# ZongyueQin/SessionSimilaritySearch

Hardware: AMD Instinct MI355X
Metric: session queries/sec (higher is better)
Workload: dtype f32

## Files before the change

### sessionsimilaritysearch_amd/_lib.py

```python
from __future__ import annotations

import ctypes
import os
import subprocess
from ctypes import c_float, c_int, c_int32, c_int64, c_size_t, c_void_p

_HERE = os.path.dirname(os.path.abspath(__file__))
LIB_PATH = os.path.join(_HERE, "libsss.so")
CSRC = os.path.join(_HERE, "csrc")

_lib = None

_SIGNATURES = {
    "sss_version": (c_int, []),
    "sss_last_error": (ctypes.c_char_p, []),
    "sss_normalize_rows": (c_int, [c_void_p, c_int64, c_int, c_int64, c_float, c_int, c_void_p]),
    "sss_row_norm_max": (c_int, [c_void_p, c_int64, c_int, c_int, c_void_p, c_void_p]),
    "sss_f32_to_bf16": (c_int, [c_void_p, c_int64, c_void_p, c_void_p]),
    "sss_ip_topk_workspace_bytes": (c_size_t, [c_int64, c_int64, c_int, c_int, c_int]),
    "sss_ip_topk_state_bytes": (c_size_t, [c_int64]),
    "sss_ip_topk": (c_int, [c_void_p, c_int64, c_void_p, c_int64, c_int, c_int, c_int, c_int64, c_float,
                            c_void_p, c_void_p, c_void_p, c_void_p, c_void_p, c_size_t, c_void_p, c_size_t, c_void_p]),
    "sss_split_bf16": (c_int, [c_void_p, c_int64, c_int, c_void_p, c_void_p]),
    "sss_ip_topk_split": (c_int, [c_void_p, c_int64, c_void_p, c_void_p, c_int64, c_int, c_int, c_int64, c_float,
# ... 80 lines not shown
_SPARSE_SIGNATURES = {
    "sss_session_vectors_count": (c_int, [c_void_p, c_void_p, c_void_p, c_int64, c_int64, c_void_p, c_void_p, c_void_p]),
    "sss_session_vectors_fill": (c_int, [c_void_p, c_void_p, c_void_p, c_int64, c_int64, c_int, ctypes.c_double, c_void_p, c_void_p,
                                         c_void_p, c_void_p, c_void_p]),
    "sss_sparse_topk_workspace_bytes": (c_size_t, [c_int64, c_int64]),
    "sss_sparse_topk": (c_int, [c_void_p, c_void_p, c_void_p, c_int64, c_void_p, c_void_p, c_void_p, c_int64, c_int, c_int64,
                                c_void_p, c_void_p, c_void_p, c_size_t, c_void_p]),
}

_L2_SIGNATURES = {
    "sss_l2_row_bias": (c_int, [c_void_p, c_int64, c_int, c_void_p, c_void_p]),
    "sss_l2_topk_workspace_bytes": (c_size_t, [c_int64, c_int64, c_int, c_int, c_int]),
    "sss_l2_topk": (c_int, [c_void_p, c_int64, c_void_p, c_void_p, c_int, c_int, c_float, c_void_p, c_int64, c_int, c_int, c_int64,
                            c_float, c_void_p, c_void_p, c_void_p, c_void_p, c_void_p, c_size_t, c_void_p, c_size_t, c_void_p]),
    "sss_l2_topk_threshold_workspace_bytes": (c_size_t, [c_int64, c_int64, c_int, c_int]),
    "sss_l2_topk_threshold": (c_int, [c_void_p, c_void_p, c_int64, c_void_p, c_void_p, c_int, c_int, c_float, c_void_p, c_int64, c_int,
                                      c_int, c_int64, c_float, c_void_p, c_void_p, c_void_p, c_void_p, c_size_t, c_void_p]),
}

_L2_LONG_SIGNATURES = {
    "sss_l2_topk_long_workspace_bytes": (c_size_t, [c_int64, c_int64, c_int]),
    "sss_l2_topk_long": (c_int, [c_void_p, c_int64, c_void_p, c_void_p, c_int, c_float, c_void_p, c_int64, c_int, c_int, c_int64,
                                 c_float, c_void_p, c_void_p, c_void_p, c_void_p, c_size_t, c_void_p]),
}

_PAD_SIGNATURES = {
    "sss_pad_rows_f32": (c_int, [c_void_p, c_int64, c_int, c_int, c_void_p, c_void_p]),
    "sss_pad_scale_f16": (c_int, [c_void_p, c_int64, c_int, c_int, c_int, c_void_p, c_void_p]),
    "sss_pad_split_bf16": (c_int, [c_void_p, c_int64, c_int, c_int, c_void_p, c_void_p]),
    "sss_pad_f16_resid_max": (c_int, [c_void_p, c_void_p, c_int64, c_int, c_int, c_int, c_void_p, c_void_p]),
    "sss_pad_topk_workspace_bytes": (c_size_t, [c_int64, c_int64, c_int, c_int, c_int, c_int]),
    "sss_pad_topk": (c_int, [c_void_p, c_int64, c_void_p, c_void_p, c_int, c_int, c_float, c_void_p, c_int64, c_int, c_int, c_int,
                             c_int64, c_float, c_void_p, c_void_p, c_void_p, c_void_p, c_void_p, c_size_t, c_void_p, c_size_t,
                             c_void_p]),
    "sss_pad_topk_threshold_workspace_bytes": (c_size_t, [c_int64, c_int64, c_int, c_int, c_int]),
    "sss_pad_topk_threshold": (c_int, [c_void_p, c_void_p, c_int64, c_void_p, c_void_p, c_int, c_int, c_float, c_void_p, c_int64,
                                       c_int, c_int, c_int, c_int64, c_float, c_void_p, c_void_p, c_void_p, c_void_p, c_size_t,
                                       c_void_p]),
}

GRAPH_IGNORE_QUERY = 1
_GRAPH_SIGNATURES = {
    "sss_graph_counts_ex": (c_int, [c_void_p, c_void_p, c_void_p, c_int64, c_int, c_void_p, c_void_p, c_void_p, c_void_p]),
    "sss_graph_fill_ex": (c_int, [c_void_p, c_void_p, c_void_p, c_void_p, c_int64, c_int, c_void_p, c_void_p, c_void_p, c_void_p,
                                  c_void_p]),
}

_EVAL_SIGNATURES = {
    "sss_item_overlap": (c_int, [c_void_p, c_void_p, c_int64, c_void_p, c_void_p, c_int64, c_void_p, c_int, c_int64, c_void_p, c_void_p,
                                 c_void_p, c_void_p]),
    "sss_overlap_metrics": (c_int, [c_void_p, c_void_p, c_void_p, c_int64, c_int, c_float, c_void_p, c_void_p, c_void_p]),
}


HEADERS = {
    "sss.h": _SIGNATURES,
    "sss_sparse.h": _SPARSE_SIGNATURES,
    "sss_l2.h": _L2_SIGNATURES,
    "sss_l2_long.h": _L2_LONG_SIGNATURES,
    "sss_pad.h": _PAD_SIGNATURES,
    "sss_graph.h": _GRAPH_SIGNATURES,
    "sss_eval.h": _EVAL_SIGNATURES,
}


class LinearProblem(ctypes.Structure):
    _fields_ = [("x", c_void_p), ("ldx", c_int64), ("ids", c_void_p), ("table", c_void_p), ("xcopy", c_void_p),
                ("ld_xcopy", c_int64), ("w", c_void_p), ("ldw", c_int64), ("bias", c_void_p), ("y", c_void_p),
                ("ldy", c_int64), ("n", c_int64), ("m", c_int32), ("act", c_int32), ("post_scale", c_void_p), ("post_shift", c_void_p)]


class GraphOut(ctypes.Structure):
    _fields_ = [(n, c_void_p) for n in ("q_x", "q_batch", "q_pos", "p_x", "p_batch", "p_cnt", "rowptr_qp", "col_qp",
                                        "rowptr_pq", "col_pq", "rowptr_pp", "col_pp", "w_pp", "src_row", "pos_id")]


class LayerArgs(ctypes.Structure):
    _fields_ = [("yp", c_void_p), ("ld_yp", c_int64), ("yq", c_void_p), ("ld_yq", c_int64), ("h", c_int32), ("d_x", c_int32),
                ("rowptr_qp", c_void_p), ("col_qp", c_void_p), ("rowptr_pp", c_void_p), ("col_pp", c_void_p),
                ("w_pp", c_void_p), ("bias_qp", c_void_p), ("b_ih", c_void_p),
                ("xin_p", c_void_p), ("ld_xin", c_int64), ("out_p", c_void_p), ("ld_out_p", c_int64), ("np", c_int64),
                ("rowptr_pq", c_void_p), ("col_pq", c_void_p), ("bias_pq", c_void_p),
                ("out_q", c_void_p), ("ld_out_q", c_int64), ("nq", c_int64), ("n_self_loop", c_int64),
                ("row_p", c_void_p), ("row_q", c_void_p), ("x0_p", c_void_p), ("ld_x0_p", c_int64),
                ("xq_table", c_void_p), ("ld_xq", c_int64), ("x0_q", c_void_p), ("ld_x0_q", c_int64)]


def exported_symbols():
    return sorted(HEADERS["sss.h"])


def sparse_symbols():
    return sorted(HEADERS["sss_sparse.h"])


def l2_symbols():
    return sorted(HEADERS["sss_l2.h"])


def l2_long_symbols():
    return sorted(HEADERS["sss_l2_long.h"])


def pad_symbols():
    return sorted(HEADERS["sss_pad.h"])


def graph_symbols():
    return sorted(HEADERS["sss_graph.h"])


def eval_symbols():
    return sorted(HEADERS["sss_eval.h"])


def build(verbose: bool = False) -> str:
    cmd = ["make", "-C", CSRC, "-j4"]
    res = subprocess.run(cmd, capture_output=True, text=True)
    if res.returncode != 0:
        raise RuntimeError("building libsss.so failed:\n" + res.stdout[-4000:] + res.stderr[-4000:])
    if verbose:
        print(res.stdout)
    return LIB_PATH


def lib():
    global _lib
    if _lib is None:
        if not os.path.exists(LIB_PATH):
            raise RuntimeError(
                f"{LIB_PATH} is missing: the HIP extension is not built. Run "
                "`python -c 'import __graft_entry__ as g; g.build()'` (or `make -C "
                "sessionsimilaritysearch_amd/csrc`). There is no CPU fallback.")
        h = ctypes.CDLL(LIB_PATH)
        for table in HEADERS.values():
            for name, (res, args) in table.items():
                fn = getattr(h, name)
                fn.restype, fn.argtypes = res, args
        _lib = h
    return _lib


class SssError(RuntimeError):
    pass


def check(rc: int, what: str):
    if rc != 0:
        msg = lib().sss_last_error()
        raise SssError(f"{what} failed (rc={rc}): {msg.decode() if msg else ''}")


def stream_ptr(device=None):
    import torch
    return torch.cuda.current_stream(device).cuda_stream


def require_cuda(t, name, dtype=None):
    import torch
    if not isinstance(t, torch.Tensor) or not t.is_cuda:
        raise SssError(f"{name} must be a CUDA (HIP) tensor")
    if dtype is not None and t.dtype != dtype:
        raise SssError(f"{name} must have dtype {dtype}, got {t.dtype}")
    if not t.is_contiguous():
        raise SssError(f"{name} must be contiguous")
    return t
# ... 1 lines not shown
```

### sessionsimilaritysearch_amd/csrc/ip_topk.hip

```cpp
#include "scan.h"

namespace sss {

namespace {
constexpr int PROF_RING = 512;
struct Prof {
    bool on = false;
    int n = 0;
    hipEvent_t ev[2 * PROF_RING];
    bool made = false;
};
Prof g_prof[MAX_DEVICES];
}

extern "C" int sss_profile_enable(int on) {
    Prof& p = g_prof[current_device()];
    if (on && !p.made) {
        for (int i = 0; i < 2 * PROF_RING; ++i)
            if (hipEventCreate(&p.ev[i]) != hipSuccess) { set_error("profile_enable: hipEventCreate failed"); return SSS_EHIP; }
        p.made = true;
    }
    p.on = on != 0;
    p.n = 0;
    return SSS_OK;
// ... 48 lines not shown
    t.scan_dtype = scan_dtype; t.corpus_shift = corpus_shift; t.corpus_resid = corpus_resid; t.corpus_max_norm = corpus_max_norm;
    t.id_offset = id_offset;
    return t;
}

extern "C" size_t sss_ip_topk_state_bytes(int64_t nq) { return nq > 0 ? state_words(nq) * 4 : 0; }

extern "C" size_t sss_ip_topk_workspace_bytes(int64_t nq, int64_t n, int d, int k, int dtype) {
    if (nq <= 0 || n <= 0 || k <= 0 || !corpus_dtype_ok(dtype) || !fused_shape_ok(d, dtype)) return 0;
    return make_plan(nq, n, d, k, dtype).total_bytes;
}

static size_t ip_topk_scan_workspace_bytes(long nq, long n, int d, int k, int scan_dtype) {
    if (nq <= 0 || n <= 0 || k <= 0 || !fused_shape_ok(d, scan_dtype)) return 0;
    return make_plan(nq, n, d, k, scan_dtype).total_bytes;
}

extern "C" size_t sss_ip_topk_f16_workspace_bytes(int64_t nq, int64_t n, int d, int k) {
    return ip_topk_scan_workspace_bytes(nq, n, d, k, DT_F16);
}

extern "C" int sss_f16_shift(float amax) { return f16_shift(amax); }

static int ip_topk_impl(const char* what, const void* q, long nq, const void* c_scan, int scan_dtype, int corpus_shift,
                        float corpus_resid, const void* c_exact,
                        int exact_dtype, long n, int d, int k, long id_offset, float corpus_max_norm, float* D_out, long* I_out,
                        int* status, int* unproven_count, void* state, size_t state_bytes, void* ws, size_t ws_bytes,
                        hipStream_t st, const float* bias = nullptr, int d_row = 0) {
    const bool l2 = bias != nullptr;
    if (nq <= 0 || n <= 0 || k <= 0) { set_error("%s: nq, n, k must be positive", what); return SSS_EINVAL; }
    int rc = check_scan_source(what, exact_dtype, scan_dtype, d, false, c_scan, corpus_shift, corpus_resid, n, nq);
    if (rc) return rc;
    if (k > 500) { set_error("%s: k too large (max 500)", what); return SSS_EINVAL; }
    if ((reinterpret_cast<uintptr_t>(ws) & 255) || (reinterpret_cast<uintptr_t>(state) & 15)) {
        set_error("%s: workspace must be 256-byte aligned, state 16-byte aligned", what);
        return SSS_EINVAL;
    }
    if (!state || state_bytes < sss_ip_topk_state_bytes(nq)) { set_error("%s: state %zu < %zu bytes", what, state_bytes, sss_ip_topk_state_bytes(nq)); return SSS_EWORKSPACE; }
    const ScanPlan p = make_plan(nq, n, d, k, scan_dtype);
    if (ws_bytes < p.total_bytes) { set_error("%s: workspace %zu < %zu", what, ws_bytes, p.total_bytes); return SSS_EWORKSPACE; }
    char* w = reinterpret_cast<char*>(ws);

    ScanArgs a;
    a.Q = q; a.C = c_scan; a.nq = (int)nq; a.n = (int)n;
    a.tiles_per_split = p.tiles_per_split; a.total_tiles = p.total_tiles;
    a.S = p.S; a.G = p.G; a.J = p.J; a.Ju = p.Ju; a.cert = p.cert; a.boot = p.boot; a.append = p.append; a.cap = p.cap;
    a.tau_skip = p.tau_skip;
    unsigned* sw = reinterpret_cast<unsigned*>(state);
    a.slots = sw;
    a.cnt = sw + state_off_cnt(nq);
    a.maxlast = reinterpret_cast<unsigned long long*>(sw + state_off_maxlast(nq));
    a.cand = reinterpret_cast<unsigned long long*>(w);
    a.bias = bias; a.corpus_shift = corpus_shift;
    Prof& pr = g_prof[current_device()];
    const bool prof = pr.on && pr.n < PROF_RING;
    if (prof) (void)hipEventRecord(pr.ev[2 * pr.n], st);
    rc = launch_scan(scan_dtype, d, p.tile_rows, a, st);
    if (prof) { (void)hipEventRecord(pr.ev[2 * pr.n + 1], st); ++pr.n; }
    if (rc) return rc;

    SelectArgs s;
    s.Q = q; s.C = c_exact; s.nq = (int)nq; s.d = d; s.dtype = exact_dtype; s.scan_dtype = scan_dtype; s.corpus_shift = corpus_shift; s.corpus_resid = corpus_resid;
    s.k = k; s.K2 = p.K2; s.J = p.J; s.cap = p.cap; s.tau_skip = p.tau_skip;
    s.cand = a.cand; s.slots = a.slots; s.cnt = a.cnt; s.maxlast = a.maxlast;
    s.id_offset = id_offset; s.corpus_max_norm = corpus_max_norm;
    s.D_out = D_out; s.I_out = I_out; s.status = status; s.unproven_count = unproven_count;
    s.metric = l2 ? 1 : 0;
    s.d_row = d_row;
    rc = launch_select(s, st);
    if (rc) (void)hipMemsetAsync(state, 0, sss_ip_topk_state_bytes(nq), st);
    return rc;
}

template <class Prepare, class Select>
static int run_threshold_form(const ThrArgs& t, const void* c_scan, const ScanPlan& p, Prepare prepare, Select select, hipStream_t st,
                              const float* bias = nullptr) {
    int rc = prepare();
    if (rc) return rc;
    ScanArgs a = {};
    a.Q = t.Q; a.C = c_scan; a.nq = t.nsel; a.n = (int)t.n;
    a.tiles_per_split = p.tiles_per_split; a.total_tiles = p.total_tiles;
    a.S = p.S; a.G = p.G; a.J = 0; a.Ju = 0; a.cert = 1; a.boot = 0; a.append = 0; a.cap = p.cap;
    a.slots = nullptr; a.cnt = t.cnt; a.maxlast = nullptr;
    a.cand = const_cast<unsigned long long*>(t.cand);
    a.qsel = t.qsel; a.thr = t.thr;
    a.bias = bias; a.corpus_shift = t.corpus_shift;
    rc = launch_scan(t.scan_dtype, t.d, p.tile_rows, a, st);
    if (rc) return rc;
    return select();
}

constexpr int THR_CAP = 8192;
static size_t thr_head_bytes(long nsel) { return ((size_t)nsel * 8 + 255) & ~(size_t)255; }

extern "C" size_t sss_ip_topk_threshold_workspace_bytes(int64_t nsel, int64_t n, int d, int scan) {
    if (nsel <= 0 || n <= 0 || !fused_shape_ok(d, scan)) return 0;
    return thr_head_bytes(nsel) + make_thr_plan(nsel, n, d, scan, THR_CAP).total_bytes;
}

static int topk_threshold_impl(const char* what, const void* q, const int* qsel, long nsel, const void* c_exact, int exact_dtype,
                               const void* c_scan, int scan_dtype, int corpus_shift, float corpus_resid, long n, int d, int k,
                               long id_offset, float corpus_max_norm, float* D_out, long* I_out, int* status, void* ws, size_t ws_bytes,
                               hipStream_t st, const float* bias = nullptr, int d_row = 0) {
    if (nsel <= 0 || n <= 0 || k <= 0 || !qsel) { set_error("%s: nsel, n, k must be positive", what); return SSS_EINVAL; }
    const int rc = check_scan_source(what, exact_dtype, scan_dtype, d, false, c_scan, corpus_shift, corpus_resid, n, nsel);
    if (rc) return rc;
// ... 209 lines not shown
```

### sessionsimilaritysearch_amd/csrc/scan.h

```cpp
#pragma once
#include "elem.h"

namespace sss {

__host__ __device__ inline int f16_shift(float amax) {
    if (!(amax > 0.f) || !(amax <= 3.4028234663852886e38f)) return 0;
    int e;
    (void)frexpf(amax, &e);
    return 13 - e;
}

constexpr int KP = 16;
constexpr int WG_QUERIES = 256;
constexpr int MAX_SLOTS = 128;
constexpr int SLOT_STRIDE = MAX_SLOTS;
constexpr unsigned ORD_NEG_INF = 0x007FFFFFu;
constexpr double ULP32_REL = 2.4e-7;
constexpr double ULP32_MIN = 1e-44;

static inline int pow2_at_least(int x) { int p = 64; while (p < x) p <<= 1; return p; }

static inline bool long_shape_ok(int d, int exact_dtype, int scan_dtype) {
    return d > 0 && d % 64 == 0 && d * elem_bytes(exact_dtype) <= 16384 && scan_pair_ok(exact_dtype, scan_dtype, true);
}

__device__ __forceinline__ double l2_chain_step(double acc, double q, double c) {
    const double dl = __dsub_rn(q, c);
    return __dadd_rn(acc, __dmul_rn(dl, dl));
}

static inline size_t state_off_cnt(long nq) { return (size_t)nq * MAX_SLOTS; }
static inline size_t state_off_maxlast(long nq) { return (state_off_cnt(nq) + (size_t)nq + 1) & ~(size_t)1; }
static inline size_t state_words(long nq) { return state_off_maxlast(nq) + 2 * (size_t)nq; }

struct ScanPlan {
    int G, S, L, K2, J, Ju, cert, boot, append, tile_rows;
    int tau_skip;
    int total_tiles, tiles_per_split, cap;
    size_t total_bytes;
};

ScanPlan make_plan(long nq, long n, int d, int k, int dtype);

struct ScanArgs {
    const void* Q;
    const void* C;
    int nq, n, tiles_per_split, total_tiles, S, G, J, Ju, cert, boot, append, cap;
    int tau_skip = 0;
    unsigned* slots;
    unsigned* cnt;
    unsigned long long* maxlast;
    unsigned long long* cand;
    const int* qsel = nullptr;
    const float* thr = nullptr;
    const float* bias = nullptr;
    int corpus_shift = 0;
};

ScanPlan make_thr_plan(long nsel, long n, int d, int scan_dtype, int cap);
int launch_scan(int dtype, int d, int tile_rows, const ScanArgs& a, hipStream_t st);
int launch_scan_l2(int dtype, int d, int tile_rows, const ScanArgs& a, hipStream_t st);

struct SelectArgs {
    const void* Q;
    const void* C;
    int nq, d, dtype, k, K2, J, cap;
    int tau_skip = 0;
    int scan_dtype;
    int corpus_shift;
    float corpus_resid;
    const unsigned long long* cand;
    unsigned* slots;
    unsigned* cnt;
    unsigned long long* maxlast;
    long id_offset;
    float corpus_max_norm;
    float* D_out;
    long* I_out;
    int* status;
    int* unproven_count;
    int metric = 0;
    int d_row = 0;
};

int launch_select(const SelectArgs& a, hipStream_t st);

struct ThrArgs {
    const void* Q;
    const void* C;
    const int* qsel;
    int nsel, d, dtype, k, cap;
    long n;
    int scan_dtype, corpus_shift;
    float corpus_resid, corpus_max_norm;
    long id_offset;
    float* thr;
    unsigned* cnt;
    const unsigned long long* cand;
    float* D_out;
    long* I_out;
    int* status;
    double* qb = nullptr;
    int qb_ready = 0;
    int keep = 0;
    int metric = 0;
    int d_row = 0;
};
int launch_thr_prepare(const ThrArgs& a, hipStream_t st);
int launch_select_all(const ThrArgs& a, hipStream_t st);
// ... 18 lines not shown
```

### sessionsimilaritysearch_amd/csrc/scan.hip

```cpp
#include "scan_kernel.h"

namespace sss {

__device__ unsigned g_boot_expired;

extern "C" int sss_scan_boot_expired(int reset) {
    unsigned v = 0, zero = 0;
    if (hipMemcpyFromSymbol(&v, HIP_SYMBOL(g_boot_expired), sizeof(v)) != hipSuccess) { set_error("scan_boot_expired: read failed"); return SSS_EHIP; }
    if (reset && hipMemcpyToSymbol(HIP_SYMBOL(g_boot_expired), &zero, sizeof(zero)) != hipSuccess) { set_error("scan_boot_expired: reset failed"); return SSS_EHIP; }
    return (int)(v > 0x7fffffffu ? 0x7fffffffu : v);
}

int current_device() {
    int dev = 0;
    (void)hipGetDevice(&dev);
    return dev < 0 || dev >= MAX_DEVICES ? 0 : dev;
}

static int pick_splits(long n, int G, int tr) {
    int S = (256 / G) & ~7;
    if (S < 8) S = 8;
    while (S > 8 && (long)S * tr > n) S -= 8;
    return S;
}

constexpr int TR256_MIN_TILES = 24;

static size_t align256(size_t v) { return (v + 255) & ~(size_t)255; }

static ScanPlan make_plan_for(long nq, long n, int d, int k, int dtype, bool want_append);

static bool append_form_fits() {
    static int cached[MAX_DEVICES] = {};
    const int dev = current_device();
    if (cached[dev] == 0) {
        constexpr int lds = 2 * 128 * 256 + 8 * 2048;
        const void* fn = reinterpret_cast<const void*>(&k_scan<256, 128, DT_F16, 8, false, true>);
        int blocks = 0, cus = 0;
        bool ok = hipFuncSetAttribute(fn, hipFuncAttributeMaxDynamicSharedMemorySize, lds) == hipSuccess &&
                  hipOccupancyMaxActiveBlocksPerMultiprocessor(&blocks, fn, 512, lds) == hipSuccess &&
                  hipDeviceGetAttribute(&cus, hipDeviceAttributeMultiprocessorCount, dev) == hipSuccess;
        (void)hipGetLastError();
        cached[dev] = (ok && blocks >= 2 && cus >= 256) ? 1 : 2;
    }
    return cached[dev] == 1;
}

ScanPlan make_plan(long nq, long n, int d, int k, int dtype) {
    const int rb = d * elem_bytes(dtype);
    if (rb == 256 && dtype != DT_F32 && k <= KP && append_form_fits()) {
        const ScanPlan a = make_plan_for(nq, n, d, k, dtype, true);
        if (a.append) return a;
    }
    return make_plan_for(nq, n, d, k, dtype, false);
}
static ScanPlan make_plan_for(long nq, long n, int d, int k, int dtype, bool want_append) {
    ScanPlan p;
    const int rb = d * elem_bytes(dtype);
    const int wgq = rb == 1024 ? 128 : WG_QUERIES;
    p.G = (int)((nq + wgq - 1) / wgq);
    int tr = rb <= 512 ? 128 : 64;
    int S = pick_splits(n, p.G, tr);
    if (rb == 512 && (n + (long)S * 128 - 1) / ((long)S * 128) < 48) { tr = 64; S = pick_splits(n, p.G, tr); }
    if (rb == 256 && dtype != DT_F32 && n / ((long)S * 256) >= TR256_MIN_TILES) tr = 256;
    if (want_append) {
        tr = 128;
        S = pick_splits(n, p.G, tr);
        if ((long)S * p.G > 256 || (long)2 * S * tr * 7 > n) want_append = false;
        else S *= 2;
        if (!want_append) { ScanPlan none; none.append = 0; return none; }
    }
    p.tile_rows = tr;
    p.S = S;
    p.L = 2 * S;
    p.K2 = k + 2 <= KP ? (k + 2 < 8 ? 8 : k + 2) : k <= KP ? KP : k + 12;
    if ((long)p.L * KP < p.K2) p.K2 = p.L * KP;
    p.total_tiles = (int)((n + tr - 1) / tr);
    p.tiles_per_split = (p.total_tiles + S - 1) / S;
    p.cap = p.L * KP;
    const int active_splits = (p.total_tiles + p.tiles_per_split - 1) / p.tiles_per_split;
    p.J = p.K2 <= 128 ? 16 : 64;
    p.cert = 1;
    while (p.J * p.cert < p.K2 && p.cert < KP) p.cert *= 2;
    p.Ju = p.J;
    p.tau_skip = (p.cert == 1 && p.J == 16) ? 16 - p.K2 : 0;
    bool classes_ok = 2 * active_splits >= p.Ju;
    if (p.cert == 1 && p.J == 16 && active_splits < 16) {
        const int zero0 = active_splits < 8 ? 8 - active_splits : 0, zero1 = active_splits < 8 ? 8 : 16 - active_splits;
        classes_ok = zero0 <= (p.tau_skip >> 1) + (p.tau_skip & 1) && zero1 <= (p.tau_skip >> 1);
    }
    if (p.J * p.cert < p.K2 || !classes_ok) { p.J = 0; p.Ju = 0; p.tau_skip = 0; }
    p.boot = (p.J > 0 && p.cert == 1) ? 1 : 0;
    p.append = (want_append && p.boot) ? 1 : 0;
    if (want_append && !p.append) return p;
    if (p.append) p.cap = 2048;
    p.total_bytes = align256((size_t)nq * p.cap * 8);
    return p;
}

ScanPlan make_thr_plan(long nsel, long n, int d, int scan_dtype, int cap) {
    ScanPlan p = {};
    const int rb = d * elem_bytes(scan_dtype);
    const int wgq = rb == 1024 ? 128 : WG_QUERIES;
    p.G = (int)((nsel + wgq - 1) / wgq);
    p.tile_rows = rb <= 512 ? 128 : 64;
    p.S = pick_splits(n, p.G, p.tile_rows);
    p.L = 2 * p.S;
    p.total_tiles = (int)((n + p.tile_rows - 1) / p.tile_rows);
    p.tiles_per_split = (p.total_tiles + p.S - 1) / p.S;
    p.cap = cap;
    p.total_bytes = align256((size_t)nsel * cap * 8);
    return p;
}

int launch_scan(int dtype, int d, int tile_rows, const ScanArgs& a, hipStream_t st) {
    const int rb = d * elem_bytes(dtype);
    if (a.bias != nullptr) return launch_scan_l2(dtype, d, tile_rows, a, st);
    int rc = 1;
    with_dtype<true>(dtype, [&](auto dt) {
        constexpr int DT = decltype(dt)::value;
        rc = launch_shape<DT, 0>(rb, tile_rows, a, st);
    });
    if (rc != 1) return rc;
    set_error("scan: unsupported row size %d bytes", rb);
    return SSS_EINVAL;
}

}
```

### sessionsimilaritysearch_amd/csrc/scan_kernel.h

```cpp
#pragma once
#include "scan.h"
#include "scan_dev.h"

#ifndef SSS_STAGGER
#define SSS_STAGGER 1
#endif
#ifndef SSS_F32_SCHED
#define SSS_F32_SCHED 7
#endif

namespace sss {

extern __device__ unsigned g_boot_expired;

template <int RB, int TR, int DT, int NW, bool THR = false, bool AP = false, int MET = 0>
__global__ __launch_bounds__(NW * 64, AP ? 2 * (NW / 4) : NW / 4) void k_scan(const ScanArgs A) {
    constexpr int H = TR / 64;
    constexpr int CH = RB / 16;
    constexpr int NU = RB / 32;
    constexpr int TILE_BYTES = TR * RB;
    constexpr int LOADS_PER_WAVE = TR * CH / 64 / NW;
    constexpr int WGQ = NW * 32;
    constexpr bool PRECOMP = RB <= 512 && !AP;
    constexpr int TAU_LDS = 2 * TILE_BYTES;
    constexpr bool F32S = (SSS_F32_SCHED & 1) && DT == DT_F32 && !AP && !THR && RB == 512;
    static_assert(CH <= 64, "row longer than one LDS-DMA instruction");
    static_assert(LOADS_PER_WAVE >= 1, "a tile is at least one DMA piece per wave");
    extern __shared__ __attribute__((aligned(16))) char smem[];

    const int nq = A.nq, n = A.n, S = A.S, G = A.G, J = A.J;
    const char* __restrict__ Qb = reinterpret_cast<const char*>(A.Q);
    const char* __restrict__ Cb = reinterpret_cast<const char*>(A.C);
    const int tid = threadIdx.x;
    const int lane = tid & 63;
    const int wave = __builtin_amdgcn_readfirstlane(tid >> 6);
    const int r = lane & 31, h = lane >> 5;

    const int bid = blockIdx.x;
    const int xcd = bid & 7, slot = bid >> 3;
    const int split = xcd * (S >> 3) + slot / G;
    const int g = slot % G;

    const int q_local = wave * 32 + r;
    const int q_glob = g * WGQ + q_local;
    int q_ld = q_glob < nq ? q_glob : nq - 1;
    if constexpr (THR) q_ld = A.qsel[q_ld];
    f32x4 qc[NU];

    float ls[KP];
    int li[KP];
#pragma unroll
    for (int i = 0; i < KP; ++i) { ls[i] = -INFINITY; li[i] = -1; }
    float pend_s = -INFINITY;
    int pend_i = -1;
    constexpr int E = 4;
    float es[E];
    int ei[E];
    int ecnt = 0;
#pragma unroll
    for (int i = 0; i < E; ++i) { es[i] = -INFINITY; ei[i] = -1; }
    float tau = -INFINITY, thr = -INFINITY;
    if constexpr (THR) thr = q_glob < nq ? A.thr[q_glob] : INFINITY;
    float rmax = -INFINITY;
    float pub = -INFINITY;

    int tile_lo = split * A.tiles_per_split;
    int tile_hi = tile_lo + A.tiles_per_split;
    if (tile_hi > A.total_tiles) tile_hi = A.total_tiles;
    const int ntiles = tile_lo < tile_hi ? tile_hi - tile_lo : 0;
    const bool use_tau = !THR && J > 0;
    const bool boot = use_tau && A.boot && ntiles > 0;
    const int nb = boot ? 1 : 0;
    const int niter = ntiles + nb;
    auto tile_of = [&](int i) { return i < ntiles ? tile_lo + i : tile_lo; };
    const int skip = A.tau_skip;

    bool slots_seen = false;
    const unsigned* my_half = nullptr;
    unsigned cls_live = 0;
#ifdef SSS_EXP_NOPAIR
    const bool pair_pub = false;
#else
    const bool pair_pub = A.cert == 1;
#endif
    if (use_tau) {
        cls_live = pair_pub ? (unsigned)(split + (split >> 4)) & 15u : (unsigned)(2 * split + h) % (unsigned)A.Ju;
        my_half = A.slots + (size_t)q_ld * SLOT_STRIDE + h * (J >> 1);
    }
    auto tau_ord = [&]() -> unsigned {
        if (J == 16 && skip > 0) {
            unsigned v[8];
            load8_sc1(my_half, v);
            return tau_select16(v, skip, h);
        }
        unsigned m = 0xFFFFFFFFu;
        for (int v = 0; v < (J >> 1); v += 8) m = min(m, min8_sc1(my_half + v));
        return min(m, (unsigned)__shfl_xor((int)m, 32));
    };
    const unsigned tau_lds = (unsigned)(unsigned long)(lptr_c)smem + TAU_LDS + wave * 2048;
    auto tau_fetch = [&]() {
        int ln = lane;
        asm volatile("" : "+v"(ln));
#pragma unroll
        for (int j = 0; j < 2; ++j) {
            int qi = g * WGQ + wave * 32 + 16 * j + (ln >> 2);
            if (qi > nq - 1) qi = nq - 1;
            const unsigned off = (unsigned)qi * (unsigned)(SLOT_STRIDE * 4) + (unsigned)(ln & 3) * 16u;
            const unsigned dst = __builtin_amdgcn_readfirstlane(tau_lds + j * 1024);
            asm volatile("s_mov_b32 m0, %1\n\ts_nop 0\n\tglobal_load_lds_dwordx4 %0, %2 sc1"
                         : : "v"(off), "s"(dst), "s"(A.slots) : "memory");
        }
    };
    auto tau_read = [&]() -> unsigned {
        const u32x4* p = reinterpret_cast<const u32x4*>(smem + TAU_LDS + wave * 2048 + r * 64 + h * 32);
        const u32x4 a = p[0], b = p[1];
        if (skip > 0) {
            unsigned v[8] = {a.x, a.y, a.z, a.w, b.x, b.y, b.z, b.w};
            return tau_select16(v, skip, h);
        }
        const unsigned m = min(min(min(a.x, a.y), min(a.z, a.w)), min(min(b.x, b.y), min(b.z, b.w)));
        return min(m, (unsigned)__shfl_xor((int)m, 32));
    };
    auto set_tau = [&](unsigned m) {
        if (m > ORD_NEG_INF) tau = fmaxf(tau, ord2f(m - 1));
        thr = AP ? tau : fmaxf(ls[KP - 1], tau);
    };
    auto publish = [&](unsigned cls) {
// ... 187 lines not shown
    auto append_block = [&](const f32x16& a, int base) {
        float q0, q1, q2, q3;
        const float m = block_max(a, q0, q1, q2, q3);
        if (__builtin_amdgcn_ballot_w64(m > thr) == 0) return;
        auto walk = [&](float qm, int j0) {
            if (__builtin_amdgcn_ballot_w64(qm > thr) == 0) return;
#pragma unroll
            for (int jj = 0; jj < 4; ++jj) {
                const int j = j0 + jj;
                const bool pass = a[j] > thr;
                if (__builtin_amdgcn_ballot_w64(pass) != 0) {
                    const bool full = pass && ecnt == E;
                    if (__builtin_amdgcn_ballot_w64(full) != 0) flush(full);
#pragma unroll
                    for (int i = E - 1; i > 0; --i) { es[i] = pass ? es[i - 1] : es[i]; ei[i] = pass ? ei[i - 1] : ei[i]; }
                    es[0] = pass ? a[j] : es[0];
                    ei[0] = pass ? base + (j & 3) + 8 * (j >> 2) : ei[0];
                    ecnt += pass ? 1 : 0;
                }
            }
        };
        walk(q0, 0); walk(q1, 4); walk(q2, 8); walk(q3, 12);
    };
    auto emit_block = [&](const f32x16& a, int base) {
        float q0, q1, q2, q3;
        const float m = block_max(a, q0, q1, q2, q3);
        if (__builtin_amdgcn_ballot_w64(m > thr) == 0) return;
#pragma unroll
        for (int j = 0; j < 16; ++j) {
            if (a[j] > thr) {
                const unsigned pos = atomicAdd(A.cnt + q_glob, 1u);
                if (pos < (unsigned)A.cap) A.cand[(size_t)q_glob * A.cap + pos] = make_key(a[j], base + (j & 3) + 8 * (j >> 2));
            }
        }
    };
    const bool two_ahead = H > 1 && niter > 1;
    if (ntiles > 0) stage(0, tile_lo);
    if (two_ahead) stage(1, tile_of(1));
    if constexpr (MET) {
        int q_shift = 0;
        load_queries<RB, DT>(Qb, q_ld, h, qc, &q_shift);
        if constexpr (DT == DT_F16) {
            const int e = A.corpus_shift + q_shift;
            bscale = ldexpf(1.f, e < -126 ? -126 : e > 127 ? 127 : e);
        }
        bias_fetch(tile_of(0));
    } else {
        load_queries<RB, DT>(Qb, q_ld, h, qc);
    }
    asm volatile("s_waitcnt vmcnt(0)" ::: "memory");
    __syncthreads();
    if constexpr (MET) bias_land();

    const int T = niter * H;
    long row0_of_step = 0;
    constexpr bool TAU_EVERY_TILE = TR >= 512;
    auto refresh_at = [&](int i) {
        if (i == 1 && boot && !TAU_EVERY_TILE) return false;
        if (TAU_EVERY_TILE || i <= 4) return true;
        const int sh = 30 - __builtin_clz(i);
        return (i & ((1 << sh) - 1)) == 0;
    };
    auto tile_top = [&](int i) {
        if (!use_tau || i == 0) return;
        if (J == 16) {
            if (!refresh_at(i)) return;
            publish(cls_live);
            tau_fetch();
            return;
        }
        const int ii = i - (wave >= 4 ? 1 : 0);
        if (ii >= 2 && (ii <= 8 || (ii & (ii - 1)) == 0 || (ii & 15) == 0)) set_tau(tau_ord());
        publish(cls_live);
    };
    auto tile_end = [&](int i) {
        const bool pre = boot && i == 0;
        if (pre) publish(cls_live);
        if constexpr (MET) { if (i + 1 < niter) bias_fetch(tile_of(i + 1)); }
        asm volatile("s_waitcnt vmcnt(0)" ::: "memory");
        if (use_tau && J == 16 && i > 0 && refresh_at(i)) { set_tau(tau_read()); slots_seen = true; }
        __syncthreads();
        if (pre) {
            unsigned m = 0;
            for (int it = 0; it < (AP ? 1024 : 24); ++it) {
                m = tau_ord();
                if (__builtin_amdgcn_ballot_w64(m == 0) == 0) break;
                __builtin_amdgcn_s_sleep(16);
            }
            if constexpr (!MET) {
                if (lane == 0 && __builtin_amdgcn_ballot_w64(m == 0 && q_glob < nq) != 0) atomicAdd(&g_boot_expired, 1u);
            }
            set_tau(m);
        }
        if constexpr (MET) bias_land();
    };
    auto score_mfma = [&](int t) {
        const int i = (int)((unsigned)t / (unsigned)H), sub = (int)((unsigned)t % (unsigned)H);
        if (sub == 0) tile_top(i);
        const int next_tile = (i + 1 < niter && !(two_ahead && i == 0)) ? tile_of(i + 1) : -1;
        mfma_sub(i & 1, sub, next_tile);
        row0_of_step = (long)tile_of(i) * TR + sub * 64;
        if (row0_of_step + 64 > n) {
#pragma unroll
            for (int j = 0; j < 16; ++j) {
                const int rr = (int)row0_of_step + 4 * h + (j & 3) + 8 * (j >> 2);
                if (rr >= n) acc0[j] = -INFINITY;
                if (rr + 32 >= n) acc1[j] = -INFINITY;
            }
        }
    };
    auto score_tree = [&]() -> float {
        float m0 = vmax3(acc0[0], acc0[1], acc0[2]), m1 = vmax3(acc1[0], acc1[1], acc1[2]);
#pragma unroll
        for (int j = 3; j < 15; j += 2) { m0 = vmax3(m0, acc0[j], acc0[j + 1]); m1 = vmax3(m1, acc1[j], acc1[j + 1]); }
        const float m = vmax3(m0, m1, acc0[15]);
        const float mm = vmax3(m, acc1[15], rmax);
        rmax = mm;
        return vmax3(m, acc1[15], acc1[15]);
    };
    const int t_live = nb * H;
    const bool defer = SSS_STAGGER && NW == 8 && (DT == DT_SPLIT || DT == DT_BF16 || DT == DT_H16 || DT == DT_I8) && wave >= 4;
    int t = 0;
    if constexpr (AP || THR) {
        t = T;
        for (int i = 0; i < niter; ++i) {
            tile_top(i);
            const int tile = tile_of(i);
            const int next_tile = (i + 1 < niter && !(two_ahead && i == 0)) ? tile_of(i + 1) : -1;
            const int row_base = tile * TR;
            const bool ragged = row_base + TR > n;
            const bool live = i >= nb;
            if constexpr (THR) {
                if (g * WGQ + wave * 32 >= nq) {
                    if (next_tile >= 0) stage((i & 1) ^ 1, next_tile);
// ... 24 lines not shown
    }
    if constexpr (F32S) {
        constexpr bool SPREAD = (SSS_F32_SCHED & 2) != 0, EARLY_TREE = (SSS_F32_SCHED & 4) != 0;
        static_assert(LOADS_PER_WAVE + 1 < NU, "a DMA piece per k-group, behind k-groups 1 .. LOADS_PER_WAVE");
        const unsigned frag_lane = (unsigned)(r * CH) * 16u;
        f32x4 nf0 = {0}, nf1 = {0};
        auto frag_ptr = [&](unsigned step_off, int u) -> const f32x4* {
            const int c = (2 * u) ^ x;
            return reinterpret_cast<const f32x4*>(smem + step_off + frag_lane + c * 16);
        };
        auto read_first = [&](unsigned step_off) { const f32x4* p = frag_ptr(step_off, 0); nf0 = p[0]; nf1 = p[32 * CH]; };
        float tm0 = -INFINITY;
        auto step = [&](int t) -> float {
            const int i = (int)((unsigned)t / (unsigned)H), sub = (int)((unsigned)t % (unsigned)H);
            const unsigned off = (unsigned)((i & 1) * TILE_BYTES + sub * (64 * RB));
            f32x4 as0[NU], as1[NU];
            as0[0] = nf0; as1[0] = nf1;
            const f32x16 zero = {0};
            if constexpr (MET) {
                float b0 = bcur[0], b1 = bcur[1];
#pragma unroll
                for (int s = 1; s < H; ++s) { b0 = sub == s ? bcur[2 * s] : b0; b1 = sub == s ? bcur[2 * s + 1] : b1; }
                acc0 = __builtin_amdgcn_mfma_f32_32x32x2f32(b0, bscale, zero, 0, 0, 0);
                acc1 = __builtin_amdgcn_mfma_f32_32x32x2f32(b1, bscale, zero, 0, 0, 0);
            } else {
                acc0 = zero; acc1 = zero;
            }
            auto fetch = [&](int u) { const f32x4* p = frag_ptr(off, u); as0[u] = p[0]; as1[u] = p[32 * CH]; };
            auto mfma8 = [&](int u) {
                const f32x4 a0 = as0[u], a1 = as1[u];
                __builtin_amdgcn_sched_barrier(0);
                acc0 = __builtin_amdgcn_mfma_f32_32x32x2f32(a0.x, qc[u].x, acc0, 0, 0, 0);
                acc1 = __builtin_amdgcn_mfma_f32_32x32x2f32(a1.x, qc[u].x, acc1, 0, 0, 0);
                acc0 = __builtin_amdgcn_mfma_f32_32x32x2f32(a0.y, qc[u].y, acc0, 0, 0, 0);
                acc1 = __builtin_amdgcn_mfma_f32_32x32x2f32(a1.y, qc[u].y, acc1, 0, 0, 0);
                acc0 = __builtin_amdgcn_mfma_f32_32x32x2f32(a0.z, qc[u].z, acc0, 0, 0, 0);
                acc1 = __builtin_amdgcn_mfma_f32_32x32x2f32(a1.z, qc[u].z, acc1, 0, 0, 0);
                acc0 = __builtin_amdgcn_mfma_f32_32x32x2f32(a0.w, qc[u].w, acc0, 0, 0, 0);
                acc1 = __builtin_amdgcn_mfma_f32_32x32x2f32(a1.w, qc[u].w, acc1, 0, 0, 0);
                __builtin_amdgcn_sched_barrier(0);
            };
            fetch(1);
            mfma8(0);
            if (sub == 0) tile_top(i);
            const int next_tile = (sub == 0 && i + 1 < niter && !(two_ahead && i == 0)) ? tile_of(i + 1) : -1;
            const long nrow0 = (long)next_tile * TR;
            const bool dma_plain = next_tile >= 0 && nrow0 + TR <= (long)n;
            const char* dma_src = Cb + (size_t)nrow0 * RB;
            const unsigned dma_dst = __builtin_amdgcn_readfirstlane(lds_base + ((i & 1) ^ 1) * TILE_BYTES + wave * LOADS_PER_WAVE * 1024);
            row0_of_step = (long)tile_of(i) * TR + sub * 64;
            const bool ragged_step = row0_of_step + 64 > n;
            const bool ends_tile = sub == H - 1 && !(boot && i == 0);
            if (next_tile >= 0 && (!dma_plain || !SPREAD)) stage((i & 1) ^ 1, next_tile);
#pragma unroll
            for (int u = 1; u < NU - 1; ++u) {
                fetch(u + 1);
                mfma8(u);
                if constexpr (SPREAD) {
                    if (u <= LOADS_PER_WAVE && dma_plain)
                        asm volatile("s_mov_b32 m0, %1\n\ts_nop 0\n\tglobal_load_lds_dwordx4 %0, %2"
                                     : : "v"(lane_off[u - 1]), "s"(dma_dst + (u - 1) * 1024), "s"(dma_src) : "memory");
                }
            }
            constexpr int u = NU - 1;
            if (ends_tile) {
                asm volatile("" : "+v"(as0[u]), "+v"(as1[u]));
                tile_end(i);
            }
            if (t + 1 < T && (sub < H - 1 || ends_tile))
                read_first(sub == H - 1 ? (unsigned)(((i + 1) & 1) * TILE_BYTES) : off + 64 * RB);
            if constexpr (!EARLY_TREE) {
                mfma8(u);
            } else {
                const f32x4 a0 = as0[u], a1 = as1[u];
                __builtin_amdgcn_sched_barrier(0);
                acc0 = __builtin_amdgcn_mfma_f32_32x32x2f32(a0.x, qc[u].x, acc0, 0, 0, 0);
                acc0 = __builtin_amdgcn_mfma_f32_32x32x2f32(a0.y, qc[u].y, acc0, 0, 0, 0);
                acc0 = __builtin_amdgcn_mfma_f32_32x32x2f32(a0.z, qc[u].z, acc0, 0, 0, 0);
                acc0 = __builtin_amdgcn_mfma_f32_32x32x2f32(a0.w, qc[u].w, acc0, 0, 0, 0);
                __builtin_amdgcn_sched_barrier(0);
                acc1 = __builtin_amdgcn_mfma_f32_32x32x2f32(a1.x, qc[u].x, acc1, 0, 0, 0);
                acc1 = __builtin_amdgcn_mfma_f32_32x32x2f32(a1.y, qc[u].y, acc1, 0, 0, 0);
                __builtin_amdgcn_sched_barrier(0);
                if (ragged_step) {
#pragma unroll
                    for (int j = 0; j < 16; ++j)
                        if ((int)row0_of_step + 4 * h + (j & 3) + 8 * (j >> 2) >= n) acc0[j] = -INFINITY;
                }
                tm0 = vmax3(acc0[0], acc0[1], acc0[2]);
#pragma unroll
                for (int j = 3; j < 15; j += 2) tm0 = vmax3(tm0, acc0[j], acc0[j + 1]);
                __builtin_amdgcn_sched_barrier(0);
                acc1 = __builtin_amdgcn_mfma_f32_32x32x2f32(a1.z, qc[u].z, acc1, 0, 0, 0);
                acc1 = __builtin_amdgcn_mfma_f32_32x32x2f32(a1.w, qc[u].w, acc1, 0, 0, 0);
                __builtin_amdgcn_sched_barrier(0);
            }
            if (ragged_step) {
#pragma unroll
                for (int j = 0; j < 16; ++j) {
                    const int rr = (int)row0_of_step + 4 * h + (j & 3) + 8 * (j >> 2);
                    if (!EARLY_TREE && rr >= n) acc0[j] = -INFINITY;
                    if (rr + 32 >= n) acc1[j] = -INFINITY;
                }
            }
            if constexpr (!EARLY_TREE) return score_tree();
            float m1 = vmax3_settled(acc1[0], acc1[1], acc1[2]);
#pragma unroll
            for (int j = 3; j < 15; j += 2) m1 = vmax3(m1, acc1[j], acc1[j + 1]);
            const float m = vmax3(tm0, m1, acc0[15]);
            rmax = vmax3(m, acc1[15], rmax);
            return vmax3(m, acc1[15], acc1[15]);
        };
        if (T > 0) read_first(0);
        while (t < T) {
            bool rare = false;
            for (; t < T; ++t) {
                const float m = step(t);
                if (t < t_live) {
                    if (t == t_live - 1) {
                        tile_end(0);
                        if (t + 1 < T) read_first((unsigned)TILE_BYTES);
                    }
                    continue;
                }
                if (__builtin_amdgcn_ballot_w64(m > thr) != 0) { rare = true; break; }
            }
            if (!rare) break;
            insert_block(acc0, (int)row0_of_step + 4 * h);
            insert_block(acc1, (int)row0_of_step + 32 + 4 * h);
            ++t;
        }
    }
    while (!F32S && t < T) {
        bool rare = false;
        for (; t < T; ++t) {
            const bool last = (unsigned)t % (unsigned)H == H - 1;
            const bool early = defer && t >= t_live;
            score_mfma(t);
            if (early && last) tile_end((int)((unsigned)t / (unsigned)H));
            const float m = score_tree();
            if (t >= t_live && __builtin_amdgcn_ballot_w64(m > thr) != 0) { rare = true; break; }
            if (!early && last) tile_end((int)((unsigned)t / (unsigned)H));
        }
        if (!rare) break;
        if constexpr (THR) {
            emit_block(acc0, (int)row0_of_step + 4 * h);
            emit_block(acc1, (int)row0_of_step + 32 + 4 * h);
        } else if constexpr (AP) {
            append_block(acc0, (int)row0_of_step + 4 * h);
            append_block(acc1, (int)row0_of_step + 32 + 4 * h);
        } else {
            insert_block(acc0, (int)row0_of_step + 4 * h);
            insert_block(acc1, (int)row0_of_step + 32 + 4 * h);
        }
        if (!defer && (unsigned)t % (unsigned)H == H - 1) tile_end((int)((unsigned)t / (unsigned)H));
        ++t;
    }
    if constexpr (THR) { flush(ecnt > 0); return; }
    if constexpr (AP) flush(ecnt > 0);
    list_insert<KP>(ls, li, pend_s, pend_i);
    if (!AP && q_glob < nq) {
        int nreal = 0;
#pragma unroll
        for (int i = 0; i < KP; ++i) nreal += li[i] >= 0 ? 1 : 0;
        if (nreal > 0) {
            const unsigned base = atomicAdd(A.cnt + q_glob, (unsigned)nreal);
            unsigned long long* dst = A.cand + (size_t)q_glob * A.cap + base;
#pragma unroll
            for (int i = 0; i < KP; ++i)
                if (i < nreal) dst[i] = make_key(ls[i], li[i]);
            if (nreal == KP) atomicMax(A.maxlast + q_glob, (unsigned long long)make_key(ls[KP - 1], li[KP - 1]));
        }
    }
}

template <int RB, int TR, int DT, int NW, int MET, bool THR, bool AP = false>
static int launch_form(const ScanArgs& a, hipStream_t st) {
    const size_t lds = 2 * (size_t)TR * RB + NW * 2048;
    const int rc = opt_in_lds(reinterpret_cast<const void*>(&k_scan<RB, TR, DT, NW, THR, AP, MET>), "k_scan", lds);
    if (rc) return rc;
    hipLaunchKernelGGL((k_scan<RB, TR, DT, NW, THR, AP, MET>), dim3(a.S * a.G), dim3(NW * 64), lds, st, a);
    return check_launch("k_scan");
}
template <int RB, int TR, int DT, int NW, int MET>
static int launch_one(const ScanArgs& a, hipStream_t st) {
    if (a.thr != nullptr) {
        if constexpr (TR == (RB <= 512 ? 128 : 64)) return launch_form<RB, TR, DT, NW, MET, true>(a, st);
        set_error("scan: threshold form not built for %d-row tiles of %d-byte rows", TR, RB);
        return SSS_EINVAL;
    }
    if (a.append) {
        if constexpr (RB == 256 && TR == 128 && DT != DT_F32) return launch_form<RB, TR, DT, NW, MET, false, true>(a, st);
        set_error("scan: append form not built for this shape");
        return SSS_EINVAL;
    }
    return launch_form<RB, TR, DT, NW, MET, false>(a, st);
}
template <int DT, int MET>
static int launch_shape(int rb, int tile_rows, const ScanArgs& a, hipStream_t st) {
    if (rb == 256) return tile_rows == 256 ? launch_one<256, 256, DT, 8, MET>(a, st) : launch_one<256, 128, DT, 8, MET>(a, st);
    if (rb == 512) return tile_rows == 128 ? launch_one<512, 128, DT, 8, MET>(a, st) : launch_one<512, 64, DT, 8, MET>(a, st);
    if (rb == 1024) return launch_one<1024, 64, DT, 4, MET>(a, st);
    return 1;
}

}
```

### sessionsimilaritysearch_amd/csrc/select.hip

```cpp
#include "select_dev.h"

namespace sss {

constexpr int FS_CAP = 2048;
constexpr int FS_K2 = 32;
constexpr int FS_COL = 16;
constexpr int SEL_MAX_K2 = 512;

__device__ __forceinline__ void clear_state(const SelectArgs& A, int q, int t, int nthreads) {
    for (int j = t; j < A.J; j += nthreads) A.slots[(size_t)q * SLOT_STRIDE + j] = 0u;
    if (t == 0) { A.cnt[q] = 0u; A.maxlast[q] = 0ull; }
}

__device__ __forceinline__ unsigned final_tau_ord(const unsigned* slots, int J, int lane, int skip) {
    if (skip > 0 && J == 16) {
        const unsigned mine = slots[lane & 15];
        int rank = 0;
#pragma unroll
        for (int j = 0; j < 16; ++j) {
            const unsigned o = (unsigned)__shfl((int)mine, j);
            rank += (o < mine || (o == mine && j < (lane & 15))) ? 1 : 0;
        }
        const unsigned long long own = __builtin_amdgcn_ballot_w64(lane < 16 && rank == skip);
        return (unsigned)__builtin_amdgcn_readlane((int)mine, __builtin_ctzll(own));
    }
    unsigned m = 0xFFFFFFFFu;
    for (int j = lane; j < J; j += 64) m = min(m, slots[j]);
#pragma unroll
    for (int o = 32; o > 0; o >>= 1) m = min(m, (unsigned)__shfl_xor((int)m, o));
    return m;
}

template <int NT>
__device__ __forceinline__ void rank_and_write(const unsigned long long* sel, const double* resc, int K2, int k,
                                               long id_offset, float* Dq, long* Iq, int t, int* s_nvalid,
                                               double* s_kth, int metric) {
    for (int c = t; c < K2; c += NT) {
        const unsigned long long key = sel[c];
        const int id = key_id(key);
        if (key == 0 || id < 0) continue;
        const float sc = (float)resc[c];
        int rank = 0;
        for (int j = 0; j < K2; ++j) {
            const int idj = key_id(sel[j]);
            if (j == c || sel[j] == 0 || idj < 0) continue;
            const float sj = (float)resc[j];
            if (sj > sc || (sj == sc && idj < id)) ++rank;
        }
        atomicAdd(s_nvalid, 1);
        if (rank < k) { Dq[rank] = out_score(sc, metric); Iq[rank] = (long)id + id_offset; }
        if (rank == k - 1) *s_kth = resc[c];
    }
}

__device__ __forceinline__ int decide_status(unsigned long long edge, unsigned long long maxlast, unsigned tau_o,
                                             int J, int nvalid, int k, double kth, double B, double unscale, double off) {
    int st = 0;
    const bool edge_real = edge != 0 && key_id(edge) >= 0;
    if (maxlast > edge) st |= 1;
    if (J > 0 && tau_o > ORD_NEG_INF) {
        if (!(edge_real && f2ord(key_score(edge)) >= tau_o)) st |= 2;
    }
    if (edge_real && nvalid >= k) {
        if (!(window_top(key_score(edge), unscale, off, B, kth) < kth)) st |= 4;
// ... 233 lines not shown
```

Measured before the change: 498,300.

## Add dynamic tile pool work-stealing to f32 scan splits

For f32 scans with 512-byte rows, the planner now gives each split a smaller static share of tiles and leaves a tail pool of tiles. Workgroups that finish their static range claim pool tiles one at a time through a global atomic counter kept in an unused slot word. The claimed index is broadcast to the workgroup through LDS. The goal is to even out load imbalance between splits at the end of the scan. In exchange it adds atomics and extra LDS traffic on the tile-end path, and the select pass must reset the counter. A plan-query entry point is also exported.

```diff
diff --git a/include/sss_scan_plan.h b/include/sss_scan_plan.h
--- /dev/null
+++ b/include/sss_scan_plan.h
@@ -0,0 +1,14 @@
+#ifndef SSS_SCAN_PLAN_H
+#define SSS_SCAN_PLAN_H
+#include <stddef.h>
+#include <stdint.h>
+#ifdef __cplusplus
+extern "C" {
+#endif
+
+int sss_scan_tile_plan(int64_t nq, int64_t n, int d, int k, int dtype, int32_t* out);
+
+#ifdef __cplusplus
+}
+#endif
+#endif
diff --git a/sessionsimilaritysearch_amd/_lib.py b/sessionsimilaritysearch_amd/_lib.py
--- a/sessionsimilaritysearch_amd/_lib.py
+++ b/sessionsimilaritysearch_amd/_lib.py
@@ -156,8 +156,13 @@
     "sss_overlap_metrics": (c_int, [c_void_p, c_void_p, c_void_p, c_int64, c_int, c_float, c_void_p, c_void_p, c_void_p]),
 }
 
+_SCAN_PLAN_SIGNATURES = {
+    "sss_scan_tile_plan": (c_int, [c_int64, c_int64, c_int, c_int, c_int, c_void_p]),
+}
+
 
 HEADERS = {
+    "sss_scan_plan.h": _SCAN_PLAN_SIGNATURES,
     "sss.h": _SIGNATURES,
     "sss_sparse.h": _SPARSE_SIGNATURES,
     "sss_l2.h": _L2_SIGNATURES,
@@ -216,6 +221,16 @@
 
 def eval_symbols():
     return sorted(HEADERS["sss_eval.h"])
+
+
+def scan_plan_symbols():
+    return sorted(HEADERS["sss_scan_plan.h"])
+
+
+def scan_tile_plan(nq: int, n: int, d: int, k: int, dtype: int = 0) -> dict:
+    out = (c_int32 * 6)()
+    check(lib().sss_scan_tile_plan(nq, n, d, k, dtype, ctypes.cast(out, c_void_p)), "sss_scan_tile_plan")
+    return dict(zip(("S", "G", "tile_rows", "tiles_per_split", "pool_first", "pool_tiles"), (int(v) for v in out)))
 
 
 def build(verbose: bool = False) -> str:
diff --git a/sessionsimilaritysearch_amd/csrc/ip_topk.hip b/sessionsimilaritysearch_amd/csrc/ip_topk.hip
--- a/sessionsimilaritysearch_amd/csrc/ip_topk.hip
+++ b/sessionsimilaritysearch_amd/csrc/ip_topk.hip
@@ -124,6 +124,7 @@
     a.maxlast = reinterpret_cast<unsigned long long*>(sw + state_off_maxlast(nq));
     a.cand = reinterpret_cast<unsigned long long*>(w);
     a.bias = bias; a.corpus_shift = corpus_shift;
+    a.pool_first = p.pool_first; a.pool_tiles = p.pool_tiles;
     Prof& pr = g_prof[current_device()];
     const bool prof = pr.on && pr.n < PROF_RING;
     if (prof) (void)hipEventRecord(pr.ev[2 * pr.n], st);
diff --git a/sessionsimilaritysearch_amd/csrc/scan.h b/sessionsimilaritysearch_amd/csrc/scan.h
--- a/sessionsimilaritysearch_amd/csrc/scan.h
+++ b/sessionsimilaritysearch_amd/csrc/scan.h
@@ -14,6 +14,7 @@
 constexpr int WG_QUERIES = 256;
 constexpr int MAX_SLOTS = 128;
 constexpr int SLOT_STRIDE = MAX_SLOTS;
+constexpr int POOL_WORD = SLOT_STRIDE - 1;
 constexpr unsigned ORD_NEG_INF = 0x007FFFFFu;
 constexpr double ULP32_REL = 2.4e-7;
 constexpr double ULP32_MIN = 1e-44;
@@ -38,6 +39,7 @@
     int tau_skip;
     int total_tiles, tiles_per_split, cap;
     size_t total_bytes;
+    int pool_first = 0, pool_tiles = 0;
 };
 
 ScanPlan make_plan(long nq, long n, int d, int k, int dtype);
@@ -55,6 +57,7 @@
     const float* thr = nullptr;
     const float* bias = nullptr;
     int corpus_shift = 0;
+    int pool_first = 0, pool_tiles = 0;
 };
 
 ScanPlan make_thr_plan(long nsel, long n, int d, int scan_dtype, int cap);
diff --git a/sessionsimilaritysearch_amd/csrc/scan.hip b/sessionsimilaritysearch_amd/csrc/scan.hip
--- a/sessionsimilaritysearch_amd/csrc/scan.hip
+++ b/sessionsimilaritysearch_amd/csrc/scan.hip
@@ -25,6 +25,7 @@
 }
 
 constexpr int TR256_MIN_TILES = 24;
+constexpr int F32_POOL_MIN_STATIC = 8;
 
 static size_t align256(size_t v) { return (v + 255) & ~(size_t)255; }
 
@@ -77,8 +78,19 @@
     if ((long)p.L * KP < p.K2) p.K2 = p.L * KP;
     p.total_tiles = (int)((n + tr - 1) / tr);
     p.tiles_per_split = (p.total_tiles + S - 1) / S;
+    int active_splits = (p.total_tiles + p.tiles_per_split - 1) / p.tiles_per_split;
+#if SSS_F32_POOL && (SSS_F32_SCHED & 1)
+    if (dtype == DT_F32 && rb == 512 && !want_append) {
+        const int B = (p.total_tiles - p.total_tiles / SSS_F32_POOL_SHARE) / S;
+        if (B >= F32_POOL_MIN_STATIC) {
+            p.tiles_per_split = B;
+            p.pool_first = S * B;
+            p.pool_tiles = p.total_tiles - S * B;
+            active_splits = S;
+        }
+    }
+#endif
     p.cap = p.L * KP;
-    const int active_splits = (p.total_tiles + p.tiles_per_split - 1) / p.tiles_per_split;
     p.J = p.K2 <= 128 ? 16 : 64;
     p.cert = 1;
     while (p.J * p.cert < p.K2 && p.cert < KP) p.cert *= 2;
@@ -113,6 +125,17 @@
     return p;
 }
 
+extern "C" int sss_scan_tile_plan(int64_t nq, int64_t n, int d, int k, int dtype, int32_t* out) {
+    if (!out) { set_error("scan_tile_plan: out is required"); return SSS_EINVAL; }
+    for (int i = 0; i < 6; ++i) out[i] = 0;
+    const Format* f = nq > 0 && n > 0 && k > 0 && d > 0 && n < (1L << 31) - 1024 && nq < (1L << 31) ? format_of(dtype) : nullptr;
+    const int rb = f ? d * elem_bytes(dtype) : 0;
+    if (rb != 256 && rb != 512 && rb != 1024) { set_error("scan_tile_plan: no fused scan of type %d for d %d", dtype, d); return SSS_EINVAL; }
+    const ScanPlan p = make_plan_for(nq, n, d, k, dtype, false);
+    out[0] = p.S; out[1] = p.G; out[2] = p.tile_rows; out[3] = p.tiles_per_split; out[4] = p.pool_first; out[5] = p.pool_tiles;
+    return SSS_OK;
+}
+
 int launch_scan(int dtype, int d, int tile_rows, const ScanArgs& a, hipStream_t st) {
     const int rb = d * elem_bytes(dtype);
     if (a.bias != nullptr) return launch_scan_l2(dtype, d, tile_rows, a, st);
diff --git a/sessionsimilaritysearch_amd/csrc/scan_kernel.h b/sessionsimilaritysearch_amd/csrc/scan_kernel.h
--- a/sessionsimilaritysearch_amd/csrc/scan_kernel.h
+++ b/sessionsimilaritysearch_amd/csrc/scan_kernel.h
@@ -7,6 +7,12 @@
 #endif
 #ifndef SSS_F32_SCHED
 #define SSS_F32_SCHED 7
+#endif
+#ifndef SSS_F32_POOL
+#define SSS_F32_POOL 1
+#endif
+#ifndef SSS_F32_POOL_SHARE
+#define SSS_F32_POOL_SHARE 16
 #endif
 
 namespace sss {
@@ -24,9 +30,12 @@
     constexpr bool PRECOMP = RB <= 512 && !AP;
     constexpr int TAU_LDS = 2 * TILE_BYTES;
     constexpr bool F32S = (SSS_F32_SCHED & 1) && DT == DT_F32 && !AP && !THR && RB == 512;
+    constexpr bool POOL = F32S && SSS_F32_POOL;
+    constexpr int POOL_LDS = TAU_LDS + NW * 2048;
     static_assert(CH <= 64, "row longer than one LDS-DMA instruction");
     static_assert(LOADS_PER_WAVE >= 1, "a tile is at least one DMA piece per wave");
     extern __shared__ __attribute__((aligned(16))) char smem[];
+    typedef unsigned __attribute__((address_space(3)))* lptr_u;
 
     const int nq = A.nq, n = A.n, S = A.S, G = A.G, J = A.J;
     const char* __restrict__ Qb = reinterpret_cast<const char*>(A.Q);
@@ -71,8 +80,17 @@
     const bool use_tau = !THR && J > 0;
     const bool boot = use_tau && A.boot && ntiles > 0;
     const int nb = boot ? 1 : 0;
-    const int niter = ntiles + nb;
-    auto tile_of = [&](int i) { return i < ntiles ? tile_lo + i : tile_lo; };
+    int niter = ntiles + nb;
+    const int niter_static = niter;
+    [[maybe_unused]] int ptile0 = -1, ptile1 = -1;
+    [[maybe_unused]] const bool pool_on = POOL && A.pool_tiles > 0;
+    [[maybe_unused]] bool pool_live = pool_on;
+    [[maybe_unused]] bool claim_now = false;
+    [[maybe_unused]] unsigned claim_v = 0, claim_w = 0;
+    auto tile_of = [&](int i) {
+        if constexpr (POOL) { if (pool_on && i >= niter_static) return (i & 1) ? ptile1 : ptile0; }
+        return i < ntiles ? tile_lo + i : tile_lo;
+    };
     const int skip = A.tau_skip;
 
     bool slots_seen = false;
@@ -366,7 +384,7 @@
     __syncthreads();
     if constexpr (MET) bias_land();
 
-    const int T = niter * H;
+    int T = niter * H;
     long row0_of_step = 0;
     constexpr bool TAU_EVERY_TILE = TR >= 512;
     auto refresh_at = [&](int i) {
@@ -393,7 +411,13 @@
         if constexpr (MET) { if (i + 1 < niter) bias_fetch(tile_of(i + 1)); }
         asm volatile("s_waitcnt vmcnt(0)" ::: "memory");
         if (use_tau && J == 16 && i > 0 && refresh_at(i)) { set_tau(tau_read()); slots_seen = true; }
+        if constexpr (POOL) {
+            if (claim_now && tid == 0) *reinterpret_cast<lptr_u>((lptr_c)smem + POOL_LDS + (i & 1) * 4) = claim_v;
+        }
         __syncthreads();
+        if constexpr (POOL) {
+            if (claim_now) claim_w = *reinterpret_cast<lptr_u>((lptr_c)smem + POOL_LDS + (i & 1) * 4);
+        }
         if (pre) {
             unsigned m = 0;
             for (int it = 0; it < (AP ? 1024 : 24); ++it) {
@@ -524,6 +548,14 @@
             const bool ragged_step = row0_of_step + 64 > n;
             const bool ends_tile = sub == H - 1 && !(boot && i == 0);
             if (next_tile >= 0 && (!dma_plain || !SPREAD)) stage((i & 1) ^ 1, next_tile);
+            if constexpr (POOL) {
+                claim_now = pool_live && ends_tile && i + 2 >= niter_static;
+                if (claim_now && tid == 0) {
+                    claim_v = 1u;
+                    asm volatile("global_atomic_add %0, %1, %0, %2 sc0"
+                                 : "+v"(claim_v) : "v"((unsigned)((g * WGQ) * SLOT_STRIDE + POOL_WORD) * 4u), "s"(A.slots) : "memory");
+                }
+            }
 #pragma unroll
             for (int u = 1; u < NU - 1; ++u) {
                 fetch(u + 1);
@@ -575,6 +607,19 @@
                     if (rr + 32 >= n) acc1[j] = -INFINITY;
                 }
             }
+            if constexpr (POOL) {
+                if (claim_now) {
+                    const unsigned c = (unsigned)__builtin_amdgcn_readfirstlane((int)claim_w);
+                    if (c < (unsigned)A.pool_tiles) {
+                        if (i & 1) ptile1 = A.pool_first + (int)c; else ptile0 = A.pool_first + (int)c;
+                        niter = i + 3;
+                        T = niter * H;
+                    } else {
+                        pool_live = false;
+                    }
+                    claim_now = false;
+                }
+            }
             if constexpr (!EARLY_TREE) return score_tree();
             float m1 = vmax3_settled(acc1[0], acc1[1], acc1[2]);
 #pragma unroll
@@ -648,7 +693,8 @@
 
 template <int RB, int TR, int DT, int NW, int MET, bool THR, bool AP = false>
 static int launch_form(const ScanArgs& a, hipStream_t st) {
-    const size_t lds = 2 * (size_t)TR * RB + NW * 2048;
+    constexpr bool POOL = (SSS_F32_SCHED & 1) && SSS_F32_POOL && DT == DT_F32 && !AP && !THR && RB == 512;
+    const size_t lds = 2 * (size_t)TR * RB + NW * 2048 + (POOL ? 16 : 0);
     const int rc = opt_in_lds(reinterpret_cast<const void*>(&k_scan<RB, TR, DT, NW, THR, AP, MET>), "k_scan", lds);
     if (rc) return rc;
     hipLaunchKernelGGL((k_scan<RB, TR, DT, NW, THR, AP, MET>), dim3(a.S * a.G), dim3(NW * 64), lds, st, a);
diff --git a/sessionsimilaritysearch_amd/csrc/select.hip b/sessionsimilaritysearch_amd/csrc/select.hip
--- a/sessionsimilaritysearch_amd/csrc/select.hip
+++ b/sessionsimilaritysearch_amd/csrc/select.hip
@@ -10,6 +10,7 @@
 __device__ __forceinline__ void clear_state(const SelectArgs& A, int q, int t, int nthreads) {
     for (int j = t; j < A.J; j += nthreads) A.slots[(size_t)q * SLOT_STRIDE + j] = 0u;
     if (t == 0) { A.cnt[q] = 0u; A.maxlast[q] = 0ull; }
+    if (t == 0 && q % WG_QUERIES == 0) A.slots[(size_t)q * SLOT_STRIDE + POOL_WORD] = 0u;
 }
 
 __device__ __forceinline__ unsigned final_tau_ord(const unsigned* slots, int J, int lane, int skip) {
```

Result: no change. 498,000 (-0.1%).
